# 3DTopia/Imagine360

Hardware: AMD Instinct MI355X
Metric: denoising steps/sec (dual-branch UNet, 16x512x1024 latent) (higher is better)
Workload: dtype bf16; 1 GPU; BASELINE cfg2: 16-frame 512x1024 equirect (pano latent 4x16x64x128 + 20 views 4x16x32x32), CFG batch 2, full-width random-init UNets, DDIM step; parallelism=single GPU, width_div=1, ddim_steps_schedule=25, outputs_finite=True

## Files before the change

imagine360_amd/csrc/abi.cpp:

```cpp
#include <hip/hip_runtime.h>
#include <stdarg.h>
#include <stdio.h>
#include <stdlib.h>
#include <atomic>
#include <mutex>
#include <vector>

#include "prof.h"

static thread_local char g_err[512] = "";

extern "C" __attribute__((visibility("hidden"))) void im360_set_error(const char* fmt, ...) {
    va_list ap;
    va_start(ap, fmt);
    vsnprintf(g_err, sizeof(g_err), fmt, ap);
    va_end(ap);
}

extern "C" __attribute__((visibility("default"))) const char* im360_last_error(void) { return g_err; }

extern "C" __attribute__((visibility("default"))) int im360_abi_version(void) { return 5; }

extern "C" __attribute__((visibility("default"))) int im360_build_flags(void) {
#ifdef IM360_ABLATE
// ... 40 lines not shown

extern "C" __attribute__((visibility("default"))) int im360_prof_collect(int kind, double* total_ms, long* launches) {
    std::lock_guard<std::mutex> lk(g_mu);
    double tot = 0.0;
    long n = 0;
    std::vector<Slot> keep;
    for (auto& s : g_used) {
        if (s.kind != kind) {
            keep.push_back(s);
            continue;
        }
        float ms = 0.f;
        if (hipEventSynchronize(s.b) == hipSuccess && hipEventElapsedTime(&ms, s.a, s.b) == hipSuccess) {
            tot += ms;
            ++n;
        }
        g_free.push_back(s);
    }
    g_used.swap(keep);
    if (total_ms) *total_ms = tot;
    if (launches) *launches = n;
    return 0;
}

namespace {
struct Knobs {
    std::atomic<int> v[im360::KNOB_COUNT];
    Knobs() {
        static const struct { int k; const char* env; int def; } init[] = {
            {im360::KNOB_ATTN_QB, "IM360_ATTN_QB", 0},       {im360::KNOB_CONV_BIG, "IM360_CONV_BIG", 1},
            {im360::KNOB_CONV_BK, "IM360_CONV_BK", 0},       {im360::KNOB_TATTN_SCALAR, "IM360_TATTN_SCALAR", 0},
            {im360::KNOB_CONV_RING, "IM360_CONV_RING", 1},    {im360::KNOB_CONV_HALO, "IM360_CONV_HALO", 0},
            {im360::KNOB_CONV_CM, "IM360_CONV_CM", 1},        {im360::KNOB_LN_PACKED, "IM360_LN_PACKED", 1},
            {im360::KNOB_RING_GROUPS, "IM360_RING_GROUPS", 0}, {im360::KNOB_ATTN_X, "IM360_ATTN_X", 3}, {im360::KNOB_ATTN_DS, "IM360_ATTN_DS", 0}, {im360::KNOB_ATTN_ONE, "IM360_ATTN_ONE", 1}, {im360::KNOB_ATTN_HG, "IM360_ATTN_HG", 0}, {im360::KNOB_CONV_SMALL, "IM360_CONV_SMALL", 2}, {im360::KNOB_ATTN_W3, "IM360_ATTN_W3", 1}, {im360::KNOB_ATTN_PIPE, "IM360_ATTN_PIPE", -1}, {im360::KNOB_CONV_STAG, "IM360_CONV_STAG", 0}, {im360::KNOB_CONV_PERSIST, "IM360_CONV_PERSIST", 0}, {im360::KNOB_GN_APPLY, "IM360_GN_APPLY", 2}, {im360::KNOB_TATTN_NT, "IM360_TATTN_NT", 0}, {im360::KNOB_NT, "IM360_NT", 1}, {im360::KNOB_G4, "IM360_G4", 0}, {im360::KNOB_GN_WGS, "IM360_GN_WGS", 0}, {im360::KNOB_CONV_KSPLIT, "IM360_CONV_KSPLIT", 1}, {im360::KNOB_FF_FUSED, "IM360_FF_FUSED", 1},
        };
        for (auto& x : v) x.store(0);
        for (auto& i : init) {
            const char* e = getenv(i.env);
            v[i.k].store(e ? atoi(e) : i.def);
        }
    }
};
Knobs g_knobs;
}

int im360::knob(int k) { return (k >= 0 && k < im360::KNOB_COUNT) ? g_knobs.v[k].load(std::memory_order_relaxed) : 0; }

extern "C" __attribute__((visibility("default"))) int im360_tuning_set(int knob, int value) {
    if (knob < 0 || knob >= im360::KNOB_COUNT) {
        im360_set_error("tuning_set: unknown knob %d", knob);
        return -1;
    }
    g_knobs.v[knob].store(value);
    return 0;
}

extern "C" __attribute__((visibility("default"))) int im360_tuning_get(int knob) { return im360::knob(knob); }
```

imagine360_amd/csrc/prof.h:

```cpp
#pragma once
namespace im360 {
enum ProfKind { PROF_ATTN = 0, PROF_TEMPORAL = 1, PROF_CONV = 2, PROF_GN_STATS = 3, PROF_GN_APPLY = 4, PROF_MISC = 5, PROF_GEMM = 6, PROF_ATTN_WARP = 7, PROF_ATTN_X2 = 8 };
struct ProfScope {
    ProfScope(int kind, void* stream);
    ~ProfScope();
    int slot_;
    void* stream_;
};
}

namespace im360 {
enum Knob { KNOB_ATTN_QB = 0, KNOB_CONV_BIG = 1, KNOB_CONV_BK = 2, KNOB_TATTN_SCALAR = 3, KNOB_CONV_RING = 4, KNOB_ATTN_HL = 5, KNOB_CONV_DBG = 6, KNOB_CONV_HALO = 7, KNOB_CONV_CM = 8, KNOB_LN_PACKED = 9, KNOB_RING_GROUPS = 10, KNOB_ATTN_X = 11, KNOB_ATTN_DS = 12, KNOB_ATTN_ONE = 13, KNOB_ATTN_DBG = 14, KNOB_ATTN_HG = 15, KNOB_CONV_SMALL = 16, KNOB_ATTN_W3 = 17, KNOB_ATTN_PIPE = 18, KNOB_CONV_STAG = 19, KNOB_CONV_PERSIST = 20, KNOB_GN_APPLY = 21, KNOB_TATTN_NT = 22, KNOB_NT = 23, KNOB_G4 = 24, KNOB_GN_WGS = 25, KNOB_CONV_KSPLIT = 26, KNOB_FF_FUSED = 27, KNOB_COUNT = 28 };
int knob(int k);
}
```

imagine360_amd/kernels.py:

```python
import ctypes
import math
import os

import torch

_LIB_PATH = os.environ.get("IM360_KERNELS_LIB") or os.path.join(os.path.dirname(os.path.abspath(__file__)), "libim360_kernels.so")
_lib = None

_I64, _F32, _INT, _PTR = ctypes.c_int64, ctypes.c_float, ctypes.c_int, ctypes.c_void_p

_SIGNATURES = {
    "im360_abi_version": (_INT, []),
    "im360_build_flags": (_INT, []),
    "im360_last_error": (ctypes.c_char_p, []),
    "im360_attn_fwd": (_INT, [_PTR] * 5 + [_I64] * 15 + [_F32, _F32, _INT, _INT, _PTR, _PTR, _PTR, _PTR, _PTR, _I64]),
    "im360_attn_fwd2": (_INT, [_PTR] * 6 + [_I64] * 19 + [_F32, _F32, _F32, _INT, _PTR]),
    "im360_temporal_attn_fwd": (_INT, [_PTR] * 4 + [_I64] * 11 + [_F32, _INT, _PTR]),
    "im360_temporal_attn_windows_fwd": (_INT, [_PTR] * 5 + [_I64] * 11 + [_PTR, _I64, _PTR, _I64, _INT, _F32, _INT, _PTR]),
    "im360_shard_pack": (_INT, [_PTR] * 2 + [_I64] * 6 + [_INT, _PTR]),
    "im360_gn_num_slabs": (_I64, [_I64] * 3),
    "im360_groupnorm_stats": (_INT, [_PTR] * 6 + [_I64] * 6 + [_F32, _INT, _PTR]),
    "im360_groupnorm_apply": (_INT, [_PTR] * 4 + [_I64] * 5 + [_INT, _INT, _PTR]),
    "im360_groupnorm_stats_cat": (_INT, [_PTR] * 7 + [_I64] * 7 + [_F32, _INT, _PTR]),
    "im360_groupnorm_fused": (_INT, [_PTR] * 7 + [_I64] * 7 + [_F32, _INT, _INT, _PTR]),
# ... 43 lines not shown
    "im360_cfg_apg_stats_windows": (_INT, [_PTR] * 4 + [_INT] + [_I64] * 4 + [_F32, _F32, _INT, _PTR, _I64, _INT, _PTR, _PTR]),
    "im360_cfg_apg_stats_windows_ring": (_INT, [_PTR] * 4 + [_INT] + [_I64] * 4 + [_F32, _F32, _INT, _PTR, _I64, _INT, _PTR, _PTR]),
    "im360_cfg_apg_scalars": (_INT, [_PTR, _I64, _I64] + [_F32] * 3 + [_INT, _F32, _F32, _PTR, _PTR, _PTR]),
    "im360_cfg_ddim_step_apg": (_INT, [_PTR] * 5 + [_I64] + [_F32] * 6 + [_INT, _F32, _F32, _PTR, _I64, _INT, _PTR, _PTR]),
    "im360_cfg_ddim_step_windows_apg": (_INT, [_PTR] * 6 + [_INT] + [_I64] * 5 + [_F32] * 6 + [_INT, _F32, _F32, _PTR, _I64, _INT, _PTR,
                                                                                              _PTR]),
    "im360_cfg_multistep_step_apg": (_INT, [_PTR] * 5 + [_I64] + [_F32] * 6 + [_INT, _F32, _F32, _PTR, _I64, _INT, _PTR, _PTR]),
    "im360_cfg_multistep_step_windows_apg": (_INT, [_PTR] * 6 + [_INT] + [_I64] * 5 + [_F32] * 6 + [_INT, _F32, _F32, _PTR, _I64, _INT,
                                                                                                   _PTR, _PTR]),
    "im360_cfg_apg_momentum_stats": (_INT, [_PTR] * 4 + [_I64, _F32, _F32, _INT, _F32, _PTR, _PTR, _I64, _INT, _PTR, _PTR]),
    "im360_cfg_apg_momentum_stats_windows": (_INT, [_PTR] * 5 + [_INT] + [_I64] * 4 + [_F32, _F32, _INT, _F32, _PTR, _PTR, _I64, _INT, _PTR,
                                                                                        _PTR]),
    "im360_cfg_apg_momentum_stats_windows_ring": (_INT, [_PTR] * 5 + [_INT] + [_I64] * 4 + [_F32, _F32, _INT, _F32, _PTR, _PTR, _I64, _INT,
                                                                                             _PTR, _PTR]),
    "im360_cfg_ddim_step_apg_momentum": (_INT, [_PTR] * 6 + [_I64] + [_F32] * 6 + [_INT, _F32, _F32, _PTR, _I64, _F32, _PTR, _INT, _PTR,
                                                                                   _PTR]),
    "im360_cfg_ddim_step_windows_apg_momentum": (_INT, [_PTR] * 7 + [_INT] + [_I64] * 5 + [_F32] * 6 + [_INT, _F32, _F32, _PTR, _I64, _F32,
                                                                                                        _PTR, _INT, _PTR, _PTR]),
    "im360_cfg_multistep_step_apg_momentum": (_INT, [_PTR] * 6 + [_I64] + [_F32] * 6 + [_INT, _F32, _F32, _PTR, _I64, _F32, _PTR, _INT,
                                                                                        _PTR, _PTR]),
    "im360_cfg_multistep_step_windows_apg_momentum": (_INT, [_PTR] * 7 + [_INT] + [_I64] * 5 + [_F32] * 6 + [_INT, _F32, _F32, _PTR, _I64,
                                                                                                             _F32, _PTR, _INT, _PTR, _PTR]),
    "im360_noise_latents": (_INT, [_PTR] * 6 + [_I64] * 5 + [_F32, _F32, _INT, _PTR]),
    "im360_keep_latents": (_INT, [_PTR] * 7 + [_I64] * 5 + [_F32, _F32, _INT, _PTR, _PTR]),
    "im360_keep_latents_release": (_INT, [_PTR] * 7 + [_I64] * 5 + [_F32, _F32, _F32, _INT, _PTR, _PTR]),
    "im360_sphere_distance2": (_INT, [_PTR] * 3 + [_I64] * 2 + [_PTR]),
    "im360_resize_pano_latent": (_INT, [_PTR] * 2 + [_I64] * 6 + [_INT, _INT, _PTR]),
    "im360_retime_pano_latent": (_INT, [_PTR] * 2 + [_I64] * 4 + [_INT, _INT, _INT, _PTR]),
    "im360_free_init_noise": (_INT, [_PTR] * 8 + [_I64] * 5 + [_F32] * 3 + [_INT, _PTR]),
    "im360_layernorm": (_INT, [_PTR] * 6 + [_I64] * 5 + [_F32, _INT, _PTR]),
    "im360_geglu": (_INT, [_PTR] * 2 + [_I64] * 2 + [_INT, _PTR]),
    "im360_linear_geglu": (_INT, [_PTR] * 4 + [_I64] * 3 + [_INT, _PTR]),
    "im360_ff_fused": (_INT, [_PTR] * 6 + [_I64, _F32] + [_PTR] * 4 + [_I64] * 4 + [_INT, _PTR]),
    "im360_softmax_rows": (_INT, [_PTR] * 2 + [_I64] * 4 + [_F32, _INT, _PTR]),
    "im360_tuning_set": (_INT, [_INT, _INT]),
    "im360_tuning_get": (_INT, [_INT]),
    "im360_prof_enable": (None, [ctypes.c_uint]),
    "im360_prof_collect": (_INT, [_INT, ctypes.POINTER(ctypes.c_double), ctypes.POINTER(ctypes.c_long)]),
}

ABI_VERSION = 5

PROF_KINDS = {"attn": 0, "temporal": 1, "conv": 2, "gn_stats": 3, "gn_apply": 4, "misc": 5, "gemm": 6, "attn_warp": 7, "attn_x2": 8}


STATS = None


SHAPES = None


def _count(kind, flops, nbytes, executed=None, shape=None):
    if STATS is not None:
        s = STATS.setdefault(kind, [0.0, 0.0, 0, 0.0])
        s[0] += flops
        s[1] += nbytes
        s[2] += 1
        s[3] += flops if executed is None else executed
    if SHAPES is not None and shape is not None:
        h = SHAPES.setdefault((kind, shape), [0, 0.0])
        h[0] += 1
        h[1] += nbytes


def exported_symbols():
    return sorted(_SIGNATURES)
# ... 588 lines not shown

FF_FUSED_SHAPE = (320, 1280)


def _ff_fused(x, w1_packed, b1_packed, c1, c2, stats, eps, w2_packed, b2, res, tag):
    _dev(x, w1_packed, b1_packed, c1, c2, stats, w2_packed, b2, res)
    k, inner = FF_FUSED_SHAPE
    m = x.numel() // k
    assert x.shape[-1] == k and x.is_contiguous() and w1_packed.shape[2] == k and w1_packed.shape[0] >= 2 * inner
    assert w2_packed.shape[2] == inner and w2_packed.shape[1] == 1 and w2_packed.shape[0] >= k and w2_packed.dtype == x.dtype
    assert res.is_contiguous() and res.numel() == x.numel() and res.dtype == x.dtype
    y = torch.empty(x.shape, dtype=x.dtype, device=x.device)
    rc = lib().im360_ff_fused(_p(x), _p(w1_packed), _p(b1_packed), _p(c1), _p(c2), _p(stats), 0 if stats is None else stats.shape[1],
                              float(eps), _p(w2_packed), _p(b2), _p(res), _p(y), m, k, inner, k, _dt(x), _stream())
    _check(rc, "im360_ff_fused")
    es = x.element_size()
    _count("gemm", 2.0 * m * k * 2 * inner + 2.0 * m * inner * k,
           es * (x.numel() + 2 * inner * k + k * inner + y.numel() + res.numel()) + (0 if stats is None else 4 * stats.numel()),
           shape=f"{tag}:{k}:{inner}")
    return y


def ff_fused(x, w1_packed, b1_packed, w2_packed, b2, res):
    return _ff_fused(x, w1_packed, b1_packed, None, None, None, 0.0, w2_packed, b2, res, "ff")


def ff_fused_ln(x, w1_packed, c1, c2, stats, eps, w2_packed, b2, res):
    assert stats.dtype == torch.float32 and stats.is_contiguous() and stats.shape[0] == x.numel() // x.shape[-1] and stats.shape[2] == 2
    for t in (c1, c2):
        assert t.dtype == torch.float32 and t.is_contiguous() and t.numel() == 2 * FF_FUSED_SHAPE[1]
    return _ff_fused(x, w1_packed, None, c1, c2, stats, eps, w2_packed, b2, res, "ff_ln")


def softmax_rows(x, scale=1.0, out=None):
    _dev(x, out)
    assert x.dim() == 2 and x.stride(1) == 1
    if out is None:
        out = torch.empty(x.shape, dtype=x.dtype, device=x.device)
    else:
        _written(out)
    rc = lib().im360_softmax_rows(_p(x), _p(out), x.shape[0], x.shape[1], x.stride(0), out.stride(0), float(scale),
                                  _dt(x), _stream())
    _check(rc, "im360_softmax_rows")
    _count("misc", 0.0, 2 * x.element_size() * x.numel())
    return out


def can_single_head_attention(d, nk):
    return d % 32 == 0 and nk % 32 == 0


def single_head_attention(q, k, v, scale):
    nq, d = q.shape
    nk = k.shape[0]
    if not can_single_head_attention(d, nk):
        raise NotImplementedError(f"single_head_attention: d={d} and Nk={nk} must be multiples of 32")
    kw = k.contiguous().reshape(nk, 1, d) if nk % 128 == 0 else pack_conv_weight(k.reshape(nk, d, 1, 1))
    s = conv2d((q * scale).contiguous().reshape(nq, 1, 1, d), kw, nk).reshape(nq, nk)
    softmax_rows(s, 1.0, out=s)
    vt = v.t().contiguous()
    vw = vt.reshape(d, 1, nk) if d % 128 == 0 else pack_conv_weight(vt.reshape(d, nk, 1, 1))
    return conv2d(s.reshape(nq, 1, 1, nk), vw, d).reshape(nq, d)


def circular_pad_w(x, pad):
    _dev(x)
# ... 552 lines not shown


def free_init_noise(x0, n1, n2, Lf, Lh, Lw, sa, sb):
    _dev(x0, n1, n2, Lf, Lh, Lw)
    dt = _dt(x0)
    if x0.dim() != 5 or x0.shape[0] != 1:
        raise ValueError(f"free_init_noise: x0 must be [1, C, F, h, w], got {list(x0.shape)}")
    _, C, F, h, w = x0.shape
    if min(C, F, h, w) < 1:
        raise ValueError(f"free_init_noise: x0 must not be empty, got {list(x0.shape)}")
    for name, n in (("n1", n1), ("n2", n2)):
        if n.dtype != torch.float32 or tuple(n.shape) != (1, F, C, h, w):
            raise ValueError(f"free_init_noise: {name} must be float32 [1, {F}, {C}, {h}, {w}], got {n.dtype} {list(n.shape)}")
    for name, L, n in (("Lf", Lf, F), ("Lh", Lh, h), ("Lw", Lw, w)):
        if L.dtype != torch.float32 or tuple(L.shape) != (n, n):
            raise ValueError(f"free_init_noise: {name} must be float32 [{n}, {n}], got {L.dtype} {list(L.shape)}")
    for name, t in (("x0", x0), ("n1", n1), ("n2", n2), ("Lf", Lf), ("Lh", Lh), ("Lw", Lw)):
        if t.device != x0.device:
            raise ValueError(f"free_init_noise: {name} is on {t.device}, x0 on {x0.device}")
        if not t.is_contiguous():
            raise ValueError(f"free_init_noise: {name} must be contiguous")
    sa, sb = float(sa), float(sb)
    if not sb > 0.0:
        raise ValueError(f"free_init_noise: sb={sb} must be positive (pure signal has no noise to replace)")
    out = torch.empty((1, F, C, h, w), dtype=torch.float32, device=x0.device)
    ws = torch.empty(2 * out.numel(), dtype=torch.float32, device=x0.device)
    rc = lib().im360_free_init_noise(_p(x0), _p(n1), _p(n2), _p(Lf), _p(Lh), _p(Lw), _p(out), _p(ws), ws.numel(), C, F, h, w, sa, sb,
                                     1.0 / sb, dt, _stream())
    _check(rc, "im360_free_init_noise")
    return out


KNOBS = {"attn_qb": 0, "conv_big": 1, "conv_bk": 2, "tattn_scalar": 3, "conv_ring": 4, "attn_hl": 5, "conv_dbg": 6, "conv_halo": 7, "conv_cm": 8, "ln_packed": 9,
         "ring_groups": 10, "attn_x": 11, "attn_ds": 12, "attn_one": 13, "attn_dbg": 14, "attn_hg": 15, "conv_small": 16, "attn_w3": 17, "attn_pipe": 18, "conv_stag": 19, "conv_persist": 20, "gn_apply": 21, "tattn_nt": 22, "nt": 23, "g4": 24, "gn_wgs": 25, "conv_ksplit": 26, "ff_fused": 27}


ATTN_PIPE_DEFAULT = -1


def ablate_build():
    return bool(lib().im360_build_flags() & 1)


def tuning_set(name, value):
    _check(lib().im360_tuning_set(KNOBS[name], int(value)), "im360_tuning_set")


def tuning_get(name):
    return lib().im360_tuning_get(KNOBS[name])


def prof_enable(kinds):
    mask = 0
    for k in kinds:
        mask |= 1 << PROF_KINDS[k]
    lib().im360_prof_enable(mask)


def prof_collect(kind):
    ms, n = ctypes.c_double(0.0), ctypes.c_long(0)
    lib().im360_prof_collect(PROF_KINDS[kind], ctypes.byref(ms), ctypes.byref(n))
    return ms.value, n.value
```

imagine360_amd/layers.py:

```python
import os

import torch
import torch.nn as nn
import torch.nn.functional as F

from . import kernels


def to_cl(x5):
    b, c, f, h, w = x5.shape
    return x5.permute(0, 2, 3, 4, 1).reshape(b * f, h, w, c).contiguous(), f


def from_cl(x, f):
    n, h, w, c = x.shape
    return x.reshape(n // f, f, h, w, c).permute(0, 4, 1, 2, 3)


class DerivedCache:

    def __init__(self):
        self._store = {}

    def get(self, key, params, build):
# ... 103 lines not shown
    y = kernels.conv2d(x.contiguous().reshape(m, 1, 1, k), wp, n, bias=bias, res=r4)
    return y.reshape(*x.shape[:-1], n)


def ln_linear(norm, weight, bias, x, stats, cache, key, post=None, post_div=1):
    n, k = weight.shape
    m = x.numel() // k
    if stats is None or not _routed(x, m, k, n) or (post is not None and post_div % 256):
        return gemm_linear(weight, bias, layer_norm(norm, x, post=post, post_div=post_div), cache=cache, key=key)

    def build():
        wg, c1, c2 = kernels.fold_layer_norm(weight, bias, norm.weight, norm.bias)
        return kernels.pack_conv_weight(wg.reshape(n, k, 1, 1).contiguous()), c1, c2

    wp, c1, c2 = cache.get(key + "_ln", (weight, bias, norm.weight, norm.bias), build)
    tab = None
    if post is not None:
        tab = cache.get(key + "_tab", (weight, post, bias, norm.weight, norm.bias), lambda: (post.float() @ weight.detach().float().t() + c2[None, :]).contiguous())
    return kernels.linear_ln(x.contiguous(), wp, c1, c2, stats, norm.eps, n, tab=tab, tab_div=post_div, tab_has_c2=tab is not None)


def _module_cache(mod):
    return mod.__dict__.setdefault("_im360_derived", DerivedCache())


def linear(lin, x, row_stats=False):
    return gemm_linear(lin.weight, lin.bias, x, cache=_module_cache(lin), row_stats=row_stats)


def linear_residual(lin, x, res, row_stats=False, gn_hw=None):
    return gemm_linear(lin.weight, lin.bias, x, res=res, cache=_module_cache(lin), row_stats=row_stats, gn_hw=gn_hw)


class GEGLU(nn.Module):

    def __init__(self, dim_in, dim_out):
        super().__init__()
        self.proj = nn.Linear(dim_in, dim_out * 2)

    def forward(self, x, ln=None, stats=None):
        two_i, k = self.proj.weight.shape
        m = x.numel() // k
        fused = (x.is_cuda or ROUTE_ON_CPU) and k % 64 == 0 and k <= GEGLU_FUSED_MAX_K and two_i % 256 == 0 and m >= ROUTE_MIN_TOKENS
        if fused and ln is not None and stats is not None:
            wp, c1p, c2p = self.packed_ln(ln)
            return kernels.linear_geglu_ln(x.contiguous(), wp, c1p, c2p, stats, ln.eps, two_i // 2)
        if ln is not None:
            x = layer_norm(ln, x)
        if fused:
            wp, bp = self.packed()
            return kernels.linear_geglu(x.contiguous(), wp, bp, two_i // 2)
        return kernels.geglu(self.proj(x))

    def packed(self):
        bias = None if self.proj.bias is None else self.proj.bias.detach()
        ps = (self.proj.weight,) if self.proj.bias is None else (self.proj.weight, self.proj.bias)
        return _module_cache(self).get("geglu", ps, lambda: kernels.pack_geglu(self.proj.weight.detach(), bias))

    def packed_ln(self, ln):
        bias = None if self.proj.bias is None else self.proj.bias.detach()

        def build():
            wg, c1, c2 = kernels.fold_layer_norm(self.proj.weight, bias, ln.weight, ln.bias)
            wp, c1p = kernels.pack_geglu(wg, c1)
            return wp, c1p.contiguous(), kernels.interleave_geglu(wg, c2)[1].contiguous()
        ps = tuple(t for t in (self.proj.weight, self.proj.bias, ln.weight, ln.bias) if t is not None)
# ... 81 lines not shown
```

imagine360_amd/unet3d.py:

```python
import math
from dataclasses import dataclass

import torch
import torch.nn as nn
import torch.nn.functional as F

from . import kernels
from .layers import (DerivedCache, FeedForward, InflatedConv3d, InflatedGroupNorm, QKVAttention, from_cl, layer_norm,
                     linear, linear_residual, ln_linear,
                     to_cl)


class Timesteps(nn.Module):

    def __init__(self, num_channels, flip_sin_to_cos=True, downscale_freq_shift=0.0):
        super().__init__()
        self.num_channels, self.flip, self.shift = num_channels, flip_sin_to_cos, downscale_freq_shift

    def forward(self, t):
        half = self.num_channels // 2
        freq = torch.exp(-math.log(10000.0) * torch.arange(half, dtype=torch.float32, device=t.device) / (half - self.shift))
        ang = t[:, None].float() * freq[None, :]
        s, c = ang.sin(), ang.cos()
        return torch.cat([c, s], dim=-1) if self.flip else torch.cat([s, c], dim=-1)


class TimestepEmbedding(nn.Module):
    def __init__(self, in_channels, time_embed_dim, out_dim=None):
        super().__init__()
        self.linear_1 = nn.Linear(in_channels, time_embed_dim)
        self.act = nn.SiLU()
        self.linear_2 = nn.Linear(time_embed_dim, out_dim or time_embed_dim)

    def forward(self, x):
        return self.linear_2(self.act(self.linear_1(x)))


class ResnetBlock3D(nn.Module):

    def __init__(self, *, in_channels, out_channels=None, temb_channels=512, groups=32, eps=1e-6, **_):
        super().__init__()
# ... 113 lines not shown

    def set_use_memory_efficient_attention_xformers(self, flag):
        self.attn1._use_memory_efficient_attention_xformers = flag
        self.attn2._use_memory_efficient_attention_xformers = flag

    def forward(self, hidden_states, encoder_hidden_states=None, frames=None, stats=None, **_):
        y = hidden_states
        a = self.attn1.self_attention(y, norm=self.norm1, stats=stats)
        y, st = self.attn1.out_proj(a, residual=y, row_stats=True)
        y, st = self.attn2(y, encoder_hidden_states, frames=frames, residual=y, norm=self.norm2, stats=st, row_stats=True)
        return self.ff(y, residual=y, ln=self.norm3, stats=st)


@dataclass
class Transformer3DModelOutput:
    sample: torch.Tensor


class Transformer3DModel(nn.Module):

    def __init__(self, num_attention_heads, attention_head_dim, in_channels, cross_attention_dim,
                 image_cross_attention_dim=1024, norm_num_groups=32, scale=1.0, num_tokens=4, **_):
        super().__init__()
        inner = num_attention_heads * attention_head_dim
        self.norm = InflatedGroupNorm(norm_num_groups, in_channels, eps=1e-6, affine=True)
        self.proj_in = nn.Linear(in_channels, inner)
        self.transformer_blocks = nn.ModuleList([BasicTransformerBlock(
            inner, num_attention_heads, attention_head_dim, cross_attention_dim, image_cross_attention_dim,
            scale=scale, num_tokens=num_tokens)])
        self.proj_out = nn.Linear(in_channels, inner)

    def forward_cl(self, x, ctx, frames):
        n, h, w, c = x.shape
        y = self.norm.forward_cl(x).reshape(n, h * w, c)
        y, st = linear(self.proj_in, y, row_stats=True)
        for blk in self.transformer_blocks:
            y = blk(y, ctx, frames=frames, stats=st)
            st = None
        out = linear_residual(self.proj_out, y, x.reshape(n, h * w, c), gn_hw=h * w)
        return kernels.carry_gn(out.reshape(n, h, w, c), out)

    def forward(self, hidden_states, encoder_hidden_states=None, timestep=None, return_dict=True):
        x, f = to_cl(hidden_states)
        out = from_cl(self.forward_cl(x, encoder_hidden_states, f), f)
        return Transformer3DModelOutput(sample=out) if return_dict else (out,)


class PositionalEncoding(nn.Module):

    def __init__(self, d_model, dropout=0.0, max_len=24):
        super().__init__()
        position = torch.arange(max_len).unsqueeze(1)
        div_term = torch.exp(torch.arange(0, d_model, 2) * (-math.log(10000.0) / d_model))
        pe = torch.zeros(1, max_len, d_model)
        pe[0, :, 0::2] = torch.sin(position * div_term)
        pe[0, :, 1::2] = torch.cos(position * div_term)
        self.register_buffer("pe", pe)


class VersatileAttention(QKVAttention):

    def __init__(self, query_dim, heads, dim_head, temporal_position_encoding=True,
                 temporal_position_encoding_max_len=24):
        super().__init__(query_dim, None, heads, dim_head)
        self.pos_encoder = PositionalEncoding(query_dim, max_len=temporal_position_encoding_max_len) \
            if temporal_position_encoding else None
        self.is_cross_attention = False
        self.frame_shard = None
# ... 57 lines not shown
class TemporalTransformerBlock(nn.Module):
    def __init__(self, dim, num_attention_heads, attention_head_dim, attention_block_types, max_len, pe=True):
        super().__init__()
        self.attention_blocks = nn.ModuleList([VersatileAttention(dim, num_attention_heads, attention_head_dim, pe, max_len)
                                               for _ in attention_block_types])
        self.norms = nn.ModuleList([nn.LayerNorm(dim) for _ in attention_block_types])
        self.ff = FeedForward(dim)
        self.ff_norm = nn.LayerNorm(dim)

    def forward(self, y, batch, frames, pixels, stats=None, frame_major=False):
        for attn, norm in zip(self.attention_blocks, self.norms):
            y, stats = attn(y, batch, frames, pixels, residual=y, norm=norm, stats=stats, row_stats=True, frame_major=frame_major)
        return self.ff(y, residual=y, ln=self.ff_norm, stats=stats)


class TemporalTransformer3DModel(nn.Module):
    def __init__(self, in_channels, num_attention_heads, attention_head_dim, num_layers, attention_block_types,
                 temporal_position_encoding, temporal_position_encoding_max_len, norm_num_groups=32):
        super().__init__()
        inner = num_attention_heads * attention_head_dim
        self.norm = InflatedGroupNorm(norm_num_groups, in_channels, eps=1e-6, affine=True)
        self.proj_in = nn.Linear(in_channels, inner)
        self.transformer_blocks = nn.ModuleList([TemporalTransformerBlock(
            inner, num_attention_heads, attention_head_dim, attention_block_types, temporal_position_encoding_max_len,
            temporal_position_encoding) for _ in range(num_layers)])
        self.proj_out = nn.Linear(in_channels, inner)

    frame_shard = None

    def forward_cl(self, x, frames):
        if self.frame_shard is not None:
            return self._forward_pixel_sharded(x, frames, self.frame_shard)
        n, h, w, c = x.shape
        y = self.norm.forward_cl(x).reshape(n * h * w, c)
        y, st = linear(self.proj_in, y, row_stats=True)
        for blk in self.transformer_blocks:
            y = blk(y, n // frames, frames, h * w, stats=st)
            st = None
        out = linear_residual(self.proj_out, y, x.reshape(n * h * w, c), gn_hw=h * w)
        return kernels.carry_gn(out.reshape(n, h, w, c), out)

    def _forward_pixel_sharded(self, x, frames, sh):
        n, h, w, c = x.shape
        b, p = n // frames, h * w
        y = self.norm.forward_cl(x)
        rows = sh.frames_to_pixels(y.reshape(b, frames, p, c))
        pp = sh.pixels_per_rank(p)
        y, st = linear(self.proj_in, rows, row_stats=True)
        for blk in self.transformer_blocks:
            y = blk(y, b, sh.total, pp, stats=st, frame_major=True)
            st = None
        y = linear(self.proj_out, y)
        back = sh.pixels_to_frames(y, b, p)
        return back.reshape(n, h, w, c) + x


class VanillaTemporalModule(nn.Module):

    def __init__(self, in_channels, num_attention_heads=8, num_transformer_block=2,
                 attention_block_types=("Temporal_Self", "Temporal_Self"), temporal_position_encoding=False,
                 temporal_position_encoding_max_len=24, temporal_attention_dim_div=1, zero_initialize=True, **_):
        super().__init__()
        self.temporal_transformer = TemporalTransformer3DModel(
            in_channels, num_attention_heads, in_channels // num_attention_heads // temporal_attention_dim_div,
            num_transformer_block, attention_block_types, temporal_position_encoding, temporal_position_encoding_max_len)
        if zero_initialize:
            for p in self.temporal_transformer.proj_out.parameters():
                nn.init.zeros_(p)
# ... 462 lines not shown
```

include/im360_kernels.h:

```cpp
#ifndef IM360_KERNELS_H
#define IM360_KERNELS_H
#include <stdint.h>
#ifdef __cplusplus
extern "C" {
#endif

int im360_abi_version(void);
int im360_build_flags(void);
const char* im360_last_error(void);

int im360_attn_fwd(const void* q, const void* k, const void* v, const void* bias, void* out,
                   int64_t B, int64_t H, int64_t Nq, int64_t Nk, int64_t D,
                   int64_t q_bs, int64_t q_rs, int64_t k_bs, int64_t k_rs,
                   int64_t v_bs, int64_t v_rs, int64_t o_bs, int64_t o_rs, int64_t bias_rs,
                   int64_t kv_group, float scale, float out_scale, int accumulate, int dtype, void* stream,
                   const void* bias_alt, const void* bias_sel,
                   const void* bias_blocks, const void* bias_blocks_alt, int64_t blocks_rs);

int im360_attn_pack_bias(const void* bias, void* out_f16, int64_t n, int dtype, void* stream);

int im360_attn_fwd2(const void* q, const void* k, const void* v, const void* k2, const void* v2, void* out,
                    int64_t B, int64_t H, int64_t Nq, int64_t Nk, int64_t Nk2, int64_t D,
                    int64_t q_bs, int64_t q_rs, int64_t k_bs, int64_t k_rs, int64_t v_bs, int64_t v_rs,
                    int64_t k2_bs, int64_t k2_rs, int64_t v2_bs, int64_t v2_rs, int64_t o_bs, int64_t o_rs,
// ... 251 lines not shown
int im360_resize_pano_latent(const void* x, void* out, int64_t C, int64_t F, int64_t h, int64_t w, int64_t H, int64_t W, int mode,
                             int dtype, void* stream);

int im360_retime_pano_latent(const void* x, void* out, int64_t C, int64_t f, int64_t F, int64_t hw, int mode, int loop, int dtype,
                             void* stream);

int im360_free_init_noise(const void* x0, const float* n1, const float* n2, const float* Lf, const float* Lh, const float* Lw, float* out,
                          float* ws, int64_t ws_elems, int64_t C, int64_t F, int64_t H, int64_t W, float sa, float sb, float inv_sb,
                          int dtype, void* stream);

int im360_layernorm(const void* x, const void* gamma, const void* beta, const void* pre, const void* post,
                    void* y, int64_t rows, int64_t C, int64_t pre_period, int64_t post_div,
                    int64_t post_mod, float eps, int dtype, void* stream);

int im360_geglu(const void* h, void* out, int64_t rows, int64_t I, int dtype, void* stream);

int im360_linear_geglu(const void* x, const void* w_packed, const void* bias_packed, void* y,
                       int64_t M, int64_t K, int64_t I, int dtype, void* stream);

int im360_linear_fwd(const void* x, const void* w_packed, const void* bias, const void* res, void* y, void* rowstats,
                     int64_t M, int64_t K, int64_t N, int dtype, void* stream, void* gn_partial);

int im360_linear_ln_fwd(const void* x, const void* w_packed, const void* c1, const void* c2, const void* rowstats,
                        int64_t rs_p, float eps, const void* tab, int64_t tab_div, int64_t tab_mod, void* y,
                        int64_t M, int64_t K, int64_t N, int dtype, void* stream);

int im360_linear_geglu_ln(const void* x, const void* w_packed, const void* c1, const void* c2, const void* rowstats,
                          int64_t rs_p, float eps, void* y, int64_t M, int64_t K, int64_t I, int dtype, void* stream);

int im360_ff_fused(const void* x, const void* w1_packed, const void* b1_packed, const void* c1, const void* c2,
                   const void* rowstats, int64_t rs_p, float eps, const void* w2_packed, const void* b2, const void* res, void* y,
                   int64_t M, int64_t K, int64_t I, int64_t N, int dtype, void* stream);

int im360_softmax_rows(const void* x, void* y, int64_t rows, int64_t cols, int64_t x_rs, int64_t y_rs,
                       float scale, int dtype, void* stream);

int im360_remap_cubic_wrap_u8(const void* img, const void* map_x, const void* map_y, const void* wtab, void* out,
                              int64_t N, int64_t M, int64_t H, int64_t W, int64_t C, int64_t h, int64_t w, void* stream);

int im360_max_rect(const uint8_t* mask, int64_t H, int64_t W, int64_t* rect);

int im360_tuning_set(int knob, int value);
int im360_tuning_get(int knob);


void im360_prof_enable(unsigned mask);
int im360_prof_collect(int kind, double* total_ms, long* launches);

#ifdef __cplusplus
}
#endif
#endif
```

Before: 3.548 steps/s.

## Fuse GroupNorm apply into the transformer proj_in linear for 320-channel blocks

```diff
diff --git a/imagine360_amd/csrc/abi.cpp b/imagine360_amd/csrc/abi.cpp
--- a/imagine360_amd/csrc/abi.cpp
+++ b/imagine360_amd/csrc/abi.cpp
@@ -96,7 +96,7 @@
             {im360::KNOB_CONV_BK, "IM360_CONV_BK", 0},       {im360::KNOB_TATTN_SCALAR, "IM360_TATTN_SCALAR", 0},
             {im360::KNOB_CONV_RING, "IM360_CONV_RING", 1},    {im360::KNOB_CONV_HALO, "IM360_CONV_HALO", 0},
             {im360::KNOB_CONV_CM, "IM360_CONV_CM", 1},        {im360::KNOB_LN_PACKED, "IM360_LN_PACKED", 1},
-            {im360::KNOB_RING_GROUPS, "IM360_RING_GROUPS", 0}, {im360::KNOB_ATTN_X, "IM360_ATTN_X", 3}, {im360::KNOB_ATTN_DS, "IM360_ATTN_DS", 0}, {im360::KNOB_ATTN_ONE, "IM360_ATTN_ONE", 1}, {im360::KNOB_ATTN_HG, "IM360_ATTN_HG", 0}, {im360::KNOB_CONV_SMALL, "IM360_CONV_SMALL", 2}, {im360::KNOB_ATTN_W3, "IM360_ATTN_W3", 1}, {im360::KNOB_ATTN_PIPE, "IM360_ATTN_PIPE", -1}, {im360::KNOB_CONV_STAG, "IM360_CONV_STAG", 0}, {im360::KNOB_CONV_PERSIST, "IM360_CONV_PERSIST", 0}, {im360::KNOB_GN_APPLY, "IM360_GN_APPLY", 2}, {im360::KNOB_TATTN_NT, "IM360_TATTN_NT", 0}, {im360::KNOB_NT, "IM360_NT", 1}, {im360::KNOB_G4, "IM360_G4", 0}, {im360::KNOB_GN_WGS, "IM360_GN_WGS", 0}, {im360::KNOB_CONV_KSPLIT, "IM360_CONV_KSPLIT", 1}, {im360::KNOB_FF_FUSED, "IM360_FF_FUSED", 1},
+            {im360::KNOB_RING_GROUPS, "IM360_RING_GROUPS", 0}, {im360::KNOB_ATTN_X, "IM360_ATTN_X", 3}, {im360::KNOB_ATTN_DS, "IM360_ATTN_DS", 0}, {im360::KNOB_ATTN_ONE, "IM360_ATTN_ONE", 1}, {im360::KNOB_ATTN_HG, "IM360_ATTN_HG", 0}, {im360::KNOB_CONV_SMALL, "IM360_CONV_SMALL", 2}, {im360::KNOB_ATTN_W3, "IM360_ATTN_W3", 1}, {im360::KNOB_ATTN_PIPE, "IM360_ATTN_PIPE", -1}, {im360::KNOB_CONV_STAG, "IM360_CONV_STAG", 0}, {im360::KNOB_CONV_PERSIST, "IM360_CONV_PERSIST", 0}, {im360::KNOB_GN_APPLY, "IM360_GN_APPLY", 2}, {im360::KNOB_TATTN_NT, "IM360_TATTN_NT", 0}, {im360::KNOB_NT, "IM360_NT", 1}, {im360::KNOB_G4, "IM360_G4", 0}, {im360::KNOB_GN_WGS, "IM360_GN_WGS", 0}, {im360::KNOB_CONV_KSPLIT, "IM360_CONV_KSPLIT", 1}, {im360::KNOB_FF_FUSED, "IM360_FF_FUSED", 1}, {im360::KNOB_GN_LINEAR, "IM360_GN_LINEAR", 1},
         };
         for (auto& x : v) x.store(0);
         for (auto& i : init) {
diff --git a/imagine360_amd/csrc/gn_linear.hip b/imagine360_amd/csrc/gn_linear.hip
--- /dev/null
+++ b/imagine360_amd/csrc/gn_linear.hip
@@ -0,0 +1,191 @@
+#include "conv_tile.h"
+#include "fma_f32.h"
+
+namespace im360 {
+namespace gnl {
+
+constexpr int BM = 128, KC = 320, NOUT = 320, NSTAGE = KC / 64, NSTEP = 3 * NSTAGE;
+constexpr int STAGE_X = BM * 128;
+constexpr int X_OFF = 0, X_BYTES = NSTAGE * STAGE_X;
+constexpr int PIECE = 64 * 128, SLOT = 2 * PIECE, NSLOT = 3;
+constexpr int RING_OFF = X_OFF + X_BYTES;
+constexpr int SS_OFF = RING_OFF + NSLOT * SLOT, SS_BYTES = 3 * 1024;
+constexpr int B_OFF = SS_OFF + SS_BYTES;
+constexpr int LDS_BYTES = B_OFF + NOUT * 2;
+static_assert(X_BYTES >= 8 * 32 * (5 * 64), "the epilogue stages its transpose in the activation tile");
+static_assert(2 * KC * 4 <= SS_BYTES && NSTEP % NSLOT == 0, "scale / shift window; a tile is a whole number of ring turns");
+static_assert(LDS_BYTES <= 160 * 1024, "LDS budget");
+
+struct Params {
+    ConvParams c;
+    const float* scale;
+    const float* shift;
+    uint32_t hw;
+};
+
+constexpr int step_pieces(int v) { return v == 2 ? 1 : 2; }
+
+template <typename T>
+__global__ __launch_bounds__(512) __attribute__((amdgpu_waves_per_eu(2, 2))) void gn_linear_kernel(Params gp) {
+    const ConvParams& p = gp.c;
+    __shared__ __attribute__((aligned(16))) char lds[LDS_BYTES];
+    const int tid = threadIdx.x, lane = tid & 63, wid = tid >> 6;
+    const int col = lane & 31, hi = lane >> 5;
+    const int wid_s = __builtin_amdgcn_readfirstlane(wid);
+    const int tq = wid_s >> 1, ch = wid_s & 1;
+    const T* xg = (const T*)p.x;
+    const uint32_t lds_u32 = __builtin_amdgcn_readfirstlane((uint32_t)(uintptr_t)(__attribute__((address_space(3))) char*)lds);
+
+    const int per_xcd = gridDim.x / 8;
+    const long ntiles = p.M / BM;
+    const long tile_step = gridDim.x;
+    long tile = (long)(blockIdx.x % 8) * per_xcd + blockIdx.x / 8;
+    if (tile >= ntiles) return;
+
+    const int srow = tid >> 3;
+    const int pd8 = ((tid & 7) ^ ((srow >> 1) & 7)) * 8;
+    const T* const wp = (const T*)p.w + (srow < 32 ? srow : 128 + srow) * KC + pd8;
+    auto dma = [&](const void* src, int off) { lds_dma16_asm(src, __builtin_amdgcn_readfirstlane(lds_u32 + (uint32_t)off)); };
+    auto issue_step = [&](auto uc, int slot) {
+        constexpr int U = decltype(uc)::value, S = U / 3, q0 = 2 * (U % 3);
+        const int base = RING_OFF + slot * SLOT + wid_s * 1024;
+        dma(wp + (q0 * 32 * KC + 64 * S), base);
+        if constexpr (step_pieces(U % 3) == 2) dma(wp + ((q0 + 1) * 32 * KC + 64 * S), base + PIECE);
+    };
+    auto issue_ss = [&](long t) {
+        const uint32_t img = (uint32_t)(t * BM) / gp.hw;
+        if (tid < 2 * (KC / 4)) dma((tid < KC / 4 ? gp.scale + tid * 4 : gp.shift + (tid - KC / 4) * 4) + (long)img * KC, SS_OFF + wid_s * 1024);
+    };
+    u32x4 raw[2][NSTAGE];
+    auto load_x = [&](long t) {
+        const T* src = xg + (t * BM + srow) * KC + pd8;
+#pragma unroll
+        for (int i = 0; i < 2; ++i)
+#pragma unroll
+            for (int s = 0; s < NSTAGE; ++s) raw[i][s] = *(const u32x4*)(src + i * (64 * KC) + 64 * s);
+    };
+    auto norm_store_x = [&]() {
+        const float* ss = (const float*)(lds + SS_OFF);
+#pragma unroll
+        for (int s = 0; s < NSTAGE; ++s) {
+            float sc[8], sh[8];
+            *(f32x4*)sc = *(const f32x4*)(ss + 64 * s + pd8);
+            *(f32x4*)(sc + 4) = *(const f32x4*)(ss + 64 * s + pd8 + 4);
+            *(f32x4*)sh = *(const f32x4*)(ss + KC + 64 * s + pd8);
+            *(f32x4*)(sh + 4) = *(const f32x4*)(ss + KC + 64 * s + pd8 + 4);
+#pragma unroll
+            for (int i = 0; i < 2; ++i) {
+                float f[8];
+                unpack8<T>(uint4{raw[i][s].x, raw[i][s].y, raw[i][s].z, raw[i][s].w}, f);
+#pragma unroll
+                for (int e = 0; e < 8; ++e) f[e] = fma_f32(f[e], sc[e], sh[e]);
+                *(uint4*)(lds + X_OFF + s * STAGE_X + i * PIECE + tid * 16) = pack8<T>(f);
+            }
+        }
+    };
+    auto wait_vm = [&](int n) {
+        if (n >= 2) asm volatile("s_waitcnt vmcnt(2)" ::: "memory");
+        else asm volatile("s_waitcnt vmcnt(1)" ::: "memory");
+    };
+
+    const int swz = (col >> 1) & 7;
+    int koff[4];
+#pragma unroll
+    for (int kc = 0; kc < 4; ++kc) koff[kc] = ((kc * 2 + hi) ^ swz) * 16;
+    const int xrow = X_OFF + (32 * tq + col) * 128;
+    const int wrow = (32 * ch + col) * 128;
+
+    if (tid < NOUT / 8) *(uint4*)(lds + B_OFF + tid * 16) = p.bias ? *(const uint4*)((const T*)p.bias + tid * 8) : uint4{0u, 0u, 0u, 0u};
+
+    issue_ss(tile);
+    load_x(tile);
+    issue_step(std::integral_constant<int, 0>{}, 0);
+    issue_step(std::integral_constant<int, 1>{}, 1);
+    asm volatile("s_waitcnt vmcnt(0)\n\ts_barrier" ::: "memory");
+    norm_store_x();
+
+    for (;;) {
+        const long m0 = tile * BM;
+        const long next = tile + tile_step;
+        const bool has_next = next < ntiles;
+
+        f32x16 oacc[5][1];
+#pragma unroll
+        for (int a = 0; a < 5; ++a)
+#pragma unroll
+            for (int r = 0; r < 16; ++r) oacc[a][0][r] = 0.f;
+
+        u32x4 xf[4];
+        static_for<NSTEP>([&](auto uc) {
+            constexpr int U = decltype(uc)::value, S = U / 3, V = U % 3;
+            constexpr int slot = U % NSLOT, slot2 = (U + 2) % NSLOT;
+            wait_vm(step_pieces((V + 1) % 3));
+            asm volatile("s_waitcnt lgkmcnt(0)\n\ts_barrier" ::: "memory");
+            if constexpr (U == 0) issue_ss(has_next ? next : tile);
+            issue_step(std::integral_constant<int, (U + 2) % NSTEP>{}, slot2);
+            const char* at = lds + RING_OFF + slot * SLOT;
+            if constexpr (V == 0) {
+#pragma unroll
+                for (int kc = 0; kc < 4; ++kc) xf[kc] = *(const u32x4*)(lds + xrow + S * STAGE_X + koff[kc]);
+            }
+            constexpr int NP = step_pieces(V), q0 = 2 * V;
+            u32x4 wf[NP][4];
+#pragma unroll
+            for (int q = 0; q < NP; ++q)
+#pragma unroll
+                for (int kc = 0; kc < 4; ++kc) wf[q][kc] = *(const u32x4*)(at + q * PIECE + wrow + koff[kc]);
+#pragma unroll
+            for (int q = 0; q < NP; ++q)
+#pragma unroll
+                for (int kc = 0; kc < 4; ++kc)
+                    oacc[q0 + q][0] = Elem<T>::mfma32(__builtin_bit_cast(uint4, wf[q][kc]), __builtin_bit_cast(uint4, xf[kc]), oacc[q0 + q][0]);
+        });
+
+        if (has_next) load_x(next);
+        __builtin_amdgcn_sched_barrier(0);
+
+        int lane_e = lane, wid_e = wid_s;
+        asm volatile("" : "+v"(lane_e), "+s"(wid_e));
+        tile_epilogue<T, 512, 1, 5, 5, true, false, false, 2, 2>(p, oacc, lds + X_OFF, m0, 0, wid_e >> 1, wid_e & 1, wid_e, lane_e,
+                                                                   (const float*)(lds + B_OFF), NOUT);
+        if (!has_next) break;
+        asm volatile("s_waitcnt lgkmcnt(0)\n\ts_barrier" ::: "memory");
+        norm_store_x();
+        tile = next;
+    }
+    asm volatile("s_waitcnt vmcnt(0)" ::: "memory");
+}
+
+}
+}
+
+extern "C" int im360_groupnorm_finalize(const void* pa, int64_t Sa, int64_t C1, const void* pb, int64_t Sb, int64_t C2, const void* gamma, const void* beta,
+                                        void* scale, void* shift, int64_t N, int64_t G, int64_t pixels, float eps, int dtype, void* stream);
+
+extern "C" __attribute__((visibility("default"))) int im360_gn_linear_fwd(const void* x, const void* partial, int64_t slabs, const void* gamma, const void* beta,
+                                   int64_t groups, float eps, const void* w_packed, const void* bias, void* y, void* rowstats, void* scale_ws,
+                                   void* shift_ws, int64_t M, int64_t hw, int64_t K, int64_t N, int dtype, void* stream) {
+    using namespace im360;
+    IM360_CHECK_ARG(x && partial && gamma && beta && w_packed && y && rowstats && scale_ws && shift_ws, "gn_linear_fwd: null pointer");
+    IM360_CHECK_ARG(M > 0 && M <= 0x7fffffffL && slabs > 0, "gn_linear_fwd: M=%ld, slabs=%ld out of range", (long)M, (long)slabs);
+    if (K != gnl::KC || N != gnl::NOUT || hw <= 0 || (hw % gnl::BM) != 0 || (M % hw) != 0 || groups <= 0 || (gnl::KC % groups) != 0) {
+        im360_set_error("gn_linear_fwd: K=%ld, N=%ld, hw=%ld, M=%ld, groups=%ld unsupported (K = N = 320, hw %% 128 == 0, M %% hw == 0, 320 %% groups == 0 only)",
+                        (long)K, (long)N, (long)hw, (long)M, (long)groups);
+        return IM360_ERR_UNSUPPORTED;
+    }
+    IM360_CHECK_ARG(((uintptr_t)x % 16) == 0 && ((uintptr_t)w_packed % 16) == 0 && ((uintptr_t)y % 16) == 0 && ((uintptr_t)bias % 16) == 0 &&
+                    ((uintptr_t)rowstats % 8) == 0 && ((uintptr_t)scale_ws % 16) == 0 && ((uintptr_t)shift_ws % 16) == 0, "gn_linear_fwd: misaligned pointer");
+    IM360_CHECK_ARG(dtype == 0 || dtype == 1, "gn_linear_fwd: dtype %d unsupported", dtype);
+    if (const int rc = im360_groupnorm_finalize(partial, slabs, K, nullptr, 0, 0, gamma, beta, scale_ws, shift_ws, M / hw, groups, hw, eps, dtype, stream); rc != IM360_OK) return rc;
+    gnl::Params gp;
+    gp.c = linear_params(x, w_packed, y, M, K, N);
+    gp.c.bias = bias; gp.c.rs_out = (float*)rowstats;
+    gp.scale = (const float*)scale_ws; gp.shift = (const float*)shift_ws; gp.hw = (uint32_t)hw;
+    ProfScope prof(PROF_GEMM, stream);
+    const unsigned grid = persistent_grid(M / gnl::BM);
+    return with_dtype(dtype, "gn_linear_fwd", [&](auto t) {
+        using T = typename decltype(t)::type;
+        hipLaunchKernelGGL((gnl::gn_linear_kernel<T>), dim3(grid), dim3(512), 0, (hipStream_t)stream, gp);
+        return im360_launch_status();
+    });
+}
diff --git a/imagine360_amd/csrc/prof.h b/imagine360_amd/csrc/prof.h
--- a/imagine360_amd/csrc/prof.h
+++ b/imagine360_amd/csrc/prof.h
@@ -10,6 +10,6 @@
 }
 
 namespace im360 {
-enum Knob { KNOB_ATTN_QB = 0, KNOB_CONV_BIG = 1, KNOB_CONV_BK = 2, KNOB_TATTN_SCALAR = 3, KNOB_CONV_RING = 4, KNOB_ATTN_HL = 5, KNOB_CONV_DBG = 6, KNOB_CONV_HALO = 7, KNOB_CONV_CM = 8, KNOB_LN_PACKED = 9, KNOB_RING_GROUPS = 10, KNOB_ATTN_X = 11, KNOB_ATTN_DS = 12, KNOB_ATTN_ONE = 13, KNOB_ATTN_DBG = 14, KNOB_ATTN_HG = 15, KNOB_CONV_SMALL = 16, KNOB_ATTN_W3 = 17, KNOB_ATTN_PIPE = 18, KNOB_CONV_STAG = 19, KNOB_CONV_PERSIST = 20, KNOB_GN_APPLY = 21, KNOB_TATTN_NT = 22, KNOB_NT = 23, KNOB_G4 = 24, KNOB_GN_WGS = 25, KNOB_CONV_KSPLIT = 26, KNOB_FF_FUSED = 27, KNOB_COUNT = 28 };
+enum Knob { KNOB_ATTN_QB = 0, KNOB_CONV_BIG = 1, KNOB_CONV_BK = 2, KNOB_TATTN_SCALAR = 3, KNOB_CONV_RING = 4, KNOB_ATTN_HL = 5, KNOB_CONV_DBG = 6, KNOB_CONV_HALO = 7, KNOB_CONV_CM = 8, KNOB_LN_PACKED = 9, KNOB_RING_GROUPS = 10, KNOB_ATTN_X = 11, KNOB_ATTN_DS = 12, KNOB_ATTN_ONE = 13, KNOB_ATTN_DBG = 14, KNOB_ATTN_HG = 15, KNOB_CONV_SMALL = 16, KNOB_ATTN_W3 = 17, KNOB_ATTN_PIPE = 18, KNOB_CONV_STAG = 19, KNOB_CONV_PERSIST = 20, KNOB_GN_APPLY = 21, KNOB_TATTN_NT = 22, KNOB_NT = 23, KNOB_G4 = 24, KNOB_GN_WGS = 25, KNOB_CONV_KSPLIT = 26, KNOB_FF_FUSED = 27, KNOB_GN_LINEAR = 28, KNOB_COUNT = 29 };
 int knob(int k);
 }
diff --git a/imagine360_amd/kernels.py b/imagine360_amd/kernels.py
--- a/imagine360_amd/kernels.py
+++ b/imagine360_amd/kernels.py
@@ -99,6 +99,7 @@
     "im360_geglu": (_INT, [_PTR] * 2 + [_I64] * 2 + [_INT, _PTR]),
     "im360_linear_geglu": (_INT, [_PTR] * 4 + [_I64] * 3 + [_INT, _PTR]),
     "im360_ff_fused": (_INT, [_PTR] * 6 + [_I64, _F32] + [_PTR] * 4 + [_I64] * 4 + [_INT, _PTR]),
+    "im360_gn_linear_fwd": (_INT, [_PTR] * 2 + [_I64] + [_PTR] * 2 + [_I64, _F32] + [_PTR] * 6 + [_I64] * 4 + [_INT, _PTR]),
     "im360_softmax_rows": (_INT, [_PTR] * 2 + [_I64] * 4 + [_F32, _INT, _PTR]),
     "im360_tuning_set": (_INT, [_INT, _INT]),
     "im360_tuning_get": (_INT, [_INT]),
@@ -753,6 +754,27 @@
     return _ff_fused(x, w1_packed, None, c1, c2, stats, eps, w2_packed, b2, res, "ff_ln")
 
 
+GN_LINEAR_SHAPE = (320, 320)
+GN_LINEAR_TILE = 128
+
+
+def gn_linear(x, gamma, beta, groups, eps, w_packed, n, bias=None):
+    _dev(x, gamma, beta, w_packed, bias)
+    N, H, W, C = x.shape
+    m, hw = N * H * W, H * W
+    assert x.is_contiguous() and gamma.dtype == x.dtype and beta.dtype == x.dtype and gamma.numel() == C
+    assert w_packed.shape[2] == C and w_packed.shape[1] == 1 and w_packed.shape[0] >= n and w_packed.dtype == x.dtype
+    pa, Sa = group_norm_partials(x)
+    y = torch.empty((m, n), dtype=x.dtype, device=x.device)
+    st = torch.empty((m, max(n // ROW_SLICE, 1), 2), dtype=torch.float32, device=x.device)
+    ws = torch.empty((2, N, C), dtype=torch.float32, device=x.device)
+    rc = lib().im360_gn_linear_fwd(_p(x), _p(pa), Sa, _p(gamma), _p(beta), groups, float(eps), _p(w_packed), _p(bias), _p(y), _p(st),
+                                   _p(ws[0]), _p(ws[1]), m, hw, C, n, _dt(x), _stream())
+    _check(rc, "im360_gn_linear_fwd")
+    _count("gemm", 2.0 * m * C * n, x.element_size() * (x.numel() + n * C + y.numel()) + 4 * st.numel(), shape=f"gn_lin+stats:{C}:{n}")
+    return y, st
+
+
 def softmax_rows(x, scale=1.0, out=None):
     _dev(x, out)
     assert x.dim() == 2 and x.stride(1) == 1
@@ -1371,7 +1393,7 @@
 
 
 KNOBS = {"attn_qb": 0, "conv_big": 1, "conv_bk": 2, "tattn_scalar": 3, "conv_ring": 4, "attn_hl": 5, "conv_dbg": 6, "conv_halo": 7, "conv_cm": 8, "ln_packed": 9,
-         "ring_groups": 10, "attn_x": 11, "attn_ds": 12, "attn_one": 13, "attn_dbg": 14, "attn_hg": 15, "conv_small": 16, "attn_w3": 17, "attn_pipe": 18, "conv_stag": 19, "conv_persist": 20, "gn_apply": 21, "tattn_nt": 22, "nt": 23, "g4": 24, "gn_wgs": 25, "conv_ksplit": 26, "ff_fused": 27}
+         "ring_groups": 10, "attn_x": 11, "attn_ds": 12, "attn_one": 13, "attn_dbg": 14, "attn_hg": 15, "conv_small": 16, "attn_w3": 17, "attn_pipe": 18, "conv_stag": 19, "conv_persist": 20, "gn_apply": 21, "tattn_nt": 22, "nt": 23, "g4": 24, "gn_wgs": 25, "conv_ksplit": 26, "ff_fused": 27, "gn_linear": 28}
 
 
 ATTN_PIPE_DEFAULT = -1
diff --git a/imagine360_amd/layers.py b/imagine360_amd/layers.py
--- a/imagine360_amd/layers.py
+++ b/imagine360_amd/layers.py
@@ -159,6 +159,21 @@
     return gemm_linear(lin.weight, lin.bias, x, res=res, cache=_module_cache(lin), row_stats=row_stats, gn_hw=gn_hw)
 
 
+def gn_linear_route(on_gpu, c, n, hw, m, single_source, knob_on):
+    return bool(on_gpu and (c, n) == kernels.GN_LINEAR_SHAPE and hw > 0 and hw % kernels.GN_LINEAR_TILE == 0 and m % hw == 0 and single_source
+                and _gemm_kernel_pays(m, c, n) and knob_on)
+
+
+def gn_linear(norm, lin, x):
+    n_img, h, w, c = x.shape
+    n = lin.weight.shape[0]
+    m = n_img * h * w
+    if gn_linear_route(x.is_cuda, c, n, h * w, m, True, True) and kernels.tuning_get("gn_linear") != 0:
+        wp = _module_cache(lin).get("w1x1", (lin.weight,), lambda: kernels.pack_conv_weight(lin.weight.detach().reshape(n, c, 1, 1)))
+        return kernels.gn_linear(x.contiguous(), norm.weight, norm.bias, norm.num_groups, norm.eps, wp, n, bias=lin.bias)
+    return linear(lin, norm.forward_cl(x).reshape(m, c), row_stats=True)
+
+
 class GEGLU(nn.Module):
 
     def __init__(self, dim_in, dim_out):
diff --git a/imagine360_amd/unet3d.py b/imagine360_amd/unet3d.py
--- a/imagine360_amd/unet3d.py
+++ b/imagine360_amd/unet3d.py
@@ -6,7 +6,7 @@
 import torch.nn.functional as F
 
 from . import kernels
-from .layers import (DerivedCache, FeedForward, InflatedConv3d, InflatedGroupNorm, QKVAttention, from_cl, layer_norm,
+from .layers import (DerivedCache, FeedForward, InflatedConv3d, InflatedGroupNorm, QKVAttention, from_cl, gn_linear, layer_norm,
                      linear, linear_residual, ln_linear,
                      to_cl)
 
@@ -186,8 +186,8 @@
 
     def forward_cl(self, x, ctx, frames):
         n, h, w, c = x.shape
-        y = self.norm.forward_cl(x).reshape(n, h * w, c)
-        y, st = linear(self.proj_in, y, row_stats=True)
+        y, st = gn_linear(self.norm, self.proj_in, x)
+        y = y.reshape(n, h * w, -1)
         for blk in self.transformer_blocks:
             y = blk(y, ctx, frames=frames, stats=st)
             st = None
@@ -311,8 +311,7 @@
         if self.frame_shard is not None:
             return self._forward_pixel_sharded(x, frames, self.frame_shard)
         n, h, w, c = x.shape
-        y = self.norm.forward_cl(x).reshape(n * h * w, c)
-        y, st = linear(self.proj_in, y, row_stats=True)
+        y, st = gn_linear(self.norm, self.proj_in, x)
         for blk in self.transformer_blocks:
             y = blk(y, n // frames, frames, h * w, stats=st)
             st = None
diff --git a/include/im360_kernels.h b/include/im360_kernels.h
--- a/include/im360_kernels.h
+++ b/include/im360_kernels.h
@@ -307,6 +307,10 @@
                    const void* rowstats, int64_t rs_p, float eps, const void* w2_packed, const void* b2, const void* res, void* y,
                    int64_t M, int64_t K, int64_t I, int64_t N, int dtype, void* stream);
 
+int im360_gn_linear_fwd(const void* x, const void* partial, int64_t slabs, const void* gamma, const void* beta, int64_t groups, float eps,
+                        const void* w_packed, const void* bias, void* y, void* rowstats, void* scale_ws, void* shift_ws,
+                        int64_t M, int64_t hw, int64_t K, int64_t N, int dtype, void* stream);
+
 int im360_softmax_rows(const void* x, void* y, int64_t rows, int64_t cols, int64_t x_rs, int64_t y_rs,
                        float scale, int dtype, void* stream);
 
```

Result: no change. 3.564 steps/s, median of 6 (+0.5%).
